# trungnt13/odin-ai

Hardware: AMD Instinct MI355X
Metric: VAE train images/sec (higher is better)
Workload: dtype f32; 1 GPU; dsprites_betavae_b256; global_batch=256, per_gpu_batch=256, parallelism=dp1, graph=True

## Files before the change

include/odin_hip.h:

```cpp
#ifndef ODIN_HIP_H
#define ODIN_HIP_H

#include <stddef.h>
#include <stdint.h>

#ifdef __cplusplus
extern "C" {
#endif

enum { ODIN_LINEAR = 0, ODIN_ELU = 1, ODIN_RELU = 2 };

typedef struct odin_conv_desc {
  int B, H, W, Cin;
  int OH, OW, Cout;
  int KH, KW, stride;
  int pad_t, pad_l;
  int act;
  int center;
  uint32_t* dy_amax;
  uint32_t* dx_amax;
  const uint32_t* x_amax;
  uint32_t* y_amax;
} odin_conv_desc;

// ... 36 lines not shown
                      const odin_conv_desc* d, void* stream);
int odin_conv2d_dgrad_first(const float* dy, const float* w, const float* aux, int aux_act, float* dx,
                            float* colsum_slab, int* colsum_rows_out, const odin_conv_desc* d, const float* x0,
                            float* wslab0, int* wslab0_rows_out, const odin_conv_desc* d0, void* stream);
int odin_dense_bwd(const float* x, const float* dy, const float* w, const float* aux, int aux_act, float* dx,
                   float* colsum_slab, int* colsum_rows_out, float* wslab, int* wslab_rows_out, int B, int K,
                   int N, int want_wgrad, int want_dgrad, const uint32_t* dy_amax, uint32_t* dx_amax, void* stream);
int odin_conv2d_reads_x_range(const odin_conv_desc* d);
int odin_deconv2d_reads_x_range(const odin_conv_desc* d);
int odin_dense_reads_x_range(int B, int K, int N);
int odin_dense_fwd_ranged(const float* x, const float* w, const float* bias, float* y, int B, int K, int N, int act,
                          const uint32_t* x_amax, uint32_t* y_amax, void* stream);
int odin_dense_bwd_ranged(const float* x, const float* dy, const float* w, const float* aux, int aux_act, float* dx,
                          float* colsum_slab, int* colsum_rows_out, float* wslab, int* wslab_rows_out, int B, int K,
                          int N, int want_wgrad, int want_dgrad, const uint32_t* dy_amax, uint32_t* dx_amax,
                          const uint32_t* x_amax, void* stream);
int odin_dense_dgrad_keeps_range(int B, int K, int N);

int odin_bernoulli_tail_fwd_bwd(int is_deconv, const float* x, const float* w, const float* bias,
                                const float* w1, const float* b1, const float* target,
                                float* logits, float* g_out, float* llk_part, int* n_part_out,
                                float* tail_slab, int* slab_rows_out, const float* scale,
                                const odin_conv_desc* d, int C1, void* stream);

int odin_dense_fwd(const float* x, const float* w, const float* bias, float* y, int B, int K,
                   int N, int act, void* stream);
int odin_dense_dgrad(const float* dy, const float* w, const float* aux, int aux_act, float* dx,
                     float* colsum_slab, int* slab_rows_out, int B, int K, int N, void* stream);
int odin_dense_wgrad(const float* x, const float* dy, float* slab, int* slab_rows_out, int B,
                     int K, int N, void* stream);

typedef struct odin_reduce_job {
  const float* src;
  float* dst;
  int n;
  int rows;
  int stride;
  int pad_;
} odin_reduce_job;
int odin_slab_reduce(const odin_reduce_job* jobs, int n_jobs, void* stream);

int odin_latent_fwd(const float* p, const float* eps, float* z, float* kl, float* fbmask, int B,
                    int D, int analytic, float free_bits, const float* capacity, void* stream);
int odin_latent_bwd(const float* p, const float* eps, const float* z, const float* dz,
                    const float* dz_extra, const float* fbmask, const float* klw,
                    const float* dloc_x, const float* dscale_x, float* dp, int B, int D,
// ... 232 lines not shown
```

odin_ai_amd/_lib.py:

```python
from __future__ import annotations

import ctypes as C
import os
from typing import Optional

_HERE = os.path.dirname(os.path.abspath(__file__))
DEFAULT_LIB = os.path.join(_HERE, 'libodin_hip.so')

ACT = {'linear': 0, 'elu': 1, 'relu': 2, None: 0}


class ConvDesc(C.Structure):
  _fields_ = [(n, C.c_int) for n in ('B', 'H', 'W', 'Cin', 'OH', 'OW', 'Cout', 'KH', 'KW',
                                     'stride', 'pad_t', 'pad_l', 'act', 'center')] + \
             [('dy_amax', C.c_void_p), ('dx_amax', C.c_void_p),
              ('x_amax', C.c_void_p), ('y_amax', C.c_void_p)]


class ReduceJob(C.Structure):
  _fields_ = [('src', C.c_void_p), ('dst', C.c_void_p), ('n', C.c_int), ('rows', C.c_int),
              ('stride', C.c_int), ('pad_', C.c_int)]


class AdamFold(C.Structure):
# ... 33 lines not shown
    'odin_dense_bwd': [P, P, P, P, I, P, P, IP, P, IP, I, I, I, I, I, P, P, P],
    'odin_dense_bwd_ranged': [P, P, P, P, I, P, P, IP, P, IP, I, I, I, I, I, P, P, P, P],
    'odin_dense_dgrad_keeps_range': [I, I, I],
    'odin_conv2d_reads_x_range': [DP],
    'odin_deconv2d_reads_x_range': [DP],
    'odin_dense_reads_x_range': [I, I, I],
    'odin_absmax': [P, C.c_size_t, P, P],
    'odin_debug_absmax_fallbacks': [],
    'odin_debug_stream_probe': [P, P, P, C.c_size_t, I, I, P],
    'odin_comm_unique_id': [P],
    'odin_comm_init': [C.POINTER(C.c_void_p), P, I, I],
    'odin_comm_destroy': [P],
    'odin_comm_library': [],
    'odin_allreduce_flat': [P, P, C.c_size_t, P],
    'odin_allgather_flat': [P, P, P, C.c_size_t, P],
    'odin_reduce_scatter_flat': [P, P, P, C.c_size_t, P],
    'odin_conv2d_fwd': [P, P, P, P, DP, P],
    'odin_conv2d_dgrad': [P, P, P, I, P, P, IP, DP, P],
    'odin_conv2d_wgrad': [P, P, P, IP, DP, P],
    'odin_deconv2d_fwd': [P, P, P, P, DP, P],
    'odin_deconv2d_dgrad': [P, P, P, I, P, P, IP, DP, P],
    'odin_deconv2d_wgrad': [P, P, P, IP, DP, P],
    'odin_bernoulli_tail_fwd_bwd': [I, P, P, P, P, P, P, P, P, P, IP, P, IP, P, DP, I, P],
    'odin_dense_fwd': [P, P, P, P, I, I, I, I, P],
    'odin_dense_fwd_ranged': [P, P, P, P, I, I, I, I, P, P, P],
    'odin_dense_dgrad': [P, P, P, I, P, P, IP, I, I, I, P],
    'odin_dense_wgrad': [P, P, P, IP, I, I, I, P],
    'odin_slab_reduce': [C.POINTER(ReduceJob), I, P],
    'odin_latent_fwd': [P, P, P, P, P, I, I, I, F, P, P],
    'odin_latent_bwd': [P, P, P, P, P, P, P, P, P, P, I, I, I, P],
    'odin_latent_tril_fwd': [P, P, P, P, P, I, I, I, F, P, P],
    'odin_latent_tril_bwd': [P, P, P, P, P, P, P, P, P, I, I, I, P],
    'odin_latent_tril_sample_logprob': [P, P, P, P, P, I, I, I, P],
    'odin_latent_block_rows': [I, I, I, I],
    'odin_latent_block_fwd': [P, P, P, P, P, C.c_uint64, P, P, P, P, P, P, P, P, I, I, I, I, I, I, F, P, P],
    'odin_latent_block_bwd': [P, P, P, P, P, P, P, P, P, P, P, P, I, P, P, P, P, P, I, I, I, I, I, P, P],
    'odin_wgrad_pair_begin': [],
    'odin_wgrad_pair_end': [],
    'odin_neck_rows': [I, I, I, I],
    'odin_neck_fwd': [C.POINTER(NeckArgs), P],
    'odin_neck_bwd': [C.POINTER(NeckArgs), P],
    'odin_elbo_bernoulli_fwd_bwd': [P, P, P, P, P, I, I, IP, P],
    'odin_elbo_bernoulli_fwd_bwd_ranged': [P, P, P, P, P, I, I, IP, P, P],
    'odin_elbo_gaussian_fwd_bwd': [P, P, P, P, P, I, I, I, I, IP, P],
    'odin_gaussian_tail_applicable': [DP, I],
    'odin_gaussian_tail_fwd_bwd': [P, P, P, P, P, P, P, P, P, IP, P, IP, P, DP, I, I, P],
# ... 155 lines not shown
```

odin_ai_amd/csrc/dispatch.hip:

```cpp
#include "odin_device.h"
#include "odin_internal.h"

namespace {

enum Family {
  GENERIC,
  SMALLC, PW1X1, SMALLDECONV, SMALLDECONV_GEN,
  FCONV_PLANES, FCONV_RING, FCONV_BLK, CONV5_BLK, TCONV_PLANES, TCONV_RING, TCONV_BLK, IGEMM_H, IGEMM,
  WGRAD_PLANES, WGRAD5_BLK, WGRAD_BLK, IGEMM_H_WGRAD, IGEMM_WGRAD,
  BWD_PLANES, BWD_BLK,
  TCONV_PLANES_FIRST,
  NOT_SERVED,
  BWD_PAIR,
  TINY_DENSE, THIN_DENSE, DENSE_H, DENSE_GEMM
};

enum { FOLDS_Y = 1, FOLDS_DX = 2, READS_X = 4 };
int traits(Family f) {
  switch (f) {
    case SMALLC: case SMALLDECONV_GEN: return FOLDS_Y;
    case SMALLDECONV: case IGEMM: case THIN_DENSE: return FOLDS_Y | FOLDS_DX;
    case FCONV_PLANES: case FCONV_BLK: case CONV5_BLK: case TCONV_PLANES: case TCONV_BLK: case IGEMM_H: case DENSE_H:
      return FOLDS_Y | FOLDS_DX | READS_X;
    case WGRAD_PLANES: case WGRAD5_BLK: case WGRAD_BLK: case IGEMM_H_WGRAD: return READS_X;
// ... 373 lines not shown
             ? 1 : 0;
}

extern "C" int odin_bernoulli_tail_fwd_bwd(int is_deconv, const float* x, const float* w, const float* bias, const float* w1,
                                           const float* b1, const float* target, float* logits, float* g_out,
                                           float* llk_part, int* n_part_out, float* tail_slab, int* slab_rows_out,
                                           const float* scale, const odin_conv_desc* d, int C1, void* stream) {
  const odin_geom g = odin_geom_fwd(d);
  const Family f = select_bernoulli_tail(is_deconv, g, d->act, C1);
  const odin_tail_args tail = {w1, b1, target, scale, logits, llk_part, tail_slab, C1};
  int rc;
  if (f == TCONV_PLANES)
    rc = odin_tconv_planes_launch(x, w, bias, nullptr, g_out, nullptr, slab_rows_out, w1, b1, target, logits, llk_part,
                                  n_part_out, tail_slab, scale, C1, d->B, d->H, d->W, d->Cin, d->Cout, 3, d->x_amax,
                                  d->dy_amax, stream);
  else if (f == TCONV_RING)
    rc = odin_tconv_ring_launch(x, w, bias, nullptr, g_out, nullptr, slab_rows_out, w1, b1, target, logits, llk_part,
                                n_part_out, tail_slab, scale, C1, d->B, d->H, d->W, d->Cout, 3, stream);
  else
    rc = odin_gather_generic(is_deconv, is_deconv ? 1 : 0, g, x, w, bias, d->act, nullptr, 0, g_out, nullptr,
                             -ODIN_MAX_COLSUM_BLOCKS, slab_rows_out, &tail, n_part_out, stream);
  return keep_range(rc, f, FOLDS_Y, g_out, (size_t)d->B * d->OH * d->OW * d->Cout, d->dy_amax, stream);
}
extern "C" int odin_bernoulli_tail_keeps_range(int is_deconv, const odin_conv_desc* d, int C1) {
  return (traits(select_bernoulli_tail(is_deconv, odin_geom_fwd(d), d->act, C1)) & FOLDS_Y) ? 1 : 0;
}

extern "C" int odin_dense_fwd(const float* x, const float* w, const float* bias, float* y, int B, int K, int N, int act,
                              void* stream) {
  return odin_dense_fwd_ranged(x, w, bias, y, B, K, N, act, nullptr, nullptr, stream);
}

extern "C" int odin_dense_fwd_ranged(const float* x, const float* w, const float* bias, float* y, int B, int K, int N,
                                     int act, const uint32_t* x_amax, uint32_t* y_amax, void* stream) {
  const Family f = select_dense_fwd(B, K, N, aligned16(x, w, y, bias));
  int rc;
  switch (f) {
    case TINY_DENSE: rc = odin_tiny_dense_fwd(x, w, bias, y, B, K, N, act, stream); break;
    case THIN_DENSE: rc = odin_thin_dense_fwd(x, w, bias, y, B, K, N, act, y_amax, stream); break;
    case DENSE_H: rc = odin_dense_h_fwd(x, w, bias, y, B, K, N, act, x_amax, y_amax, stream); break;
    case DENSE_GEMM: rc = odin_dense_gemm_fwd(x, w, bias, y, B, K, N, act, stream); break;
    default:
      rc = launch_gather(f, 0, 0, odin_geom_dense(B, K, N), x, w, bias, nullptr, 0, y, nullptr, nullptr, 1, act, nullptr,
                         y_amax, stream);
  }
  return keep_range(rc, f, FOLDS_Y, y, (size_t)B * N, y_amax, stream);
// ... 90 lines not shown
```

odin_ai_amd/csrc/odin_internal.h:

```cpp
#pragma once
#include <cstdio>
#include <cstring>
#include "../../include/odin_hip.h"

#define ODIN_MAX_SLAB_BLOCKS 256
#define ODIN_MAX_COLSUM_BLOCKS 512

#include <cstdlib>
#ifdef ODIN_DIAG
#define ODIN_DIAG_ENV(name) getenv(name)
#else
#define ODIN_DIAG_ENV(name) ((const char*)nullptr)
#endif
static inline bool odin_exact_fp32() { return getenv("ODIN_EXACT_FP32") != nullptr; }

struct odin_geom {
  int B, H, W, CI, OH, OW, CO, KH, KW, S, pt, pl, center;
};
static inline odin_geom odin_geom_fwd(const odin_conv_desc* d) {
  return {d->B, d->H, d->W, d->Cin, d->OH, d->OW, d->Cout, d->KH, d->KW, d->stride, d->pad_t, d->pad_l, d->center};
}
static inline odin_geom odin_geom_dgrad(const odin_conv_desc* d) {
  return {d->B, d->OH, d->OW, d->Cout, d->H, d->W, d->Cin, d->KH, d->KW, d->stride, d->pad_t, d->pad_l, 0};
}
// ... 95 lines not shown
                          int CO, int want_bias, int grad_u, const uint32_t* g_amax, const uint32_t* a_amax,
                          void* stream);
bool odin_conv5_blk_applicable(const odin_geom& g);
int odin_conv5_blk_launch(const float* in, const float* w, const float* bias, const float* aux, float* out,
                          float* colsum, int* rows_out, int B, int H, int W, int CI, int CO, int K, int epi, int act,
                          const uint32_t* in_amax, uint32_t* out_amax, void* stream);
bool odin_wgrad5_blk_applicable(const odin_geom& g);
int odin_wgrad5_blk_launch(const float* x, const float* dy, float* slab, int* rows_out, int B, int H, int W, int CI,
                           int CO, int K, int want_bias, const uint32_t* g_amax, const uint32_t* a_amax, void* stream);
bool odin_blk_enabled(double flop);
bool odin_blk_first();
bool odin_bwd_blk_applicable(const odin_geom& g);
int odin_bwd_blk_rows(const odin_geom& g);
int odin_bwd_blk_launch(const float* x, const float* dy, const float* w, const float* aux, int aux_act, float* dx,
                        float* colsum, float* wslab, int B, int H, int W, int Cin, int Cout, const uint32_t* dy_amax,
                        const uint32_t* x_amax, uint32_t* dx_amax, void* stream);
void odin_tconv_planes_set_stamps(void* buf);
bool odin_tconv_planes_applicable(const odin_geom& g, int epi, int C1);
int odin_tconv_planes_launch(const float* in, const float* w, const float* bias, const float* aux,
                             float* out, float* colsum, int* rows_out, const float* w1, const float* b1,
                             const float* target, float* logits, float* llk_part, int* n_part_out,
                             float* slab, const float* scale, int C1, int B, int H, int W, int CI,
                             int CO, int epi, const uint32_t* in_amax, uint32_t* out_amax, void* stream);
bool odin_tconv_planes_first_applicable(const odin_geom& g, const odin_geom& l0);
int odin_tconv_planes_first_launch(const float* in, const float* w, const float* aux, float* out, float* colsum, const float* img,
                                   int center0, float* wslab0, int* rows_out, int B, const uint32_t* in_amax,
                                   uint32_t* out_amax, void* stream);

bool odin_wgrad_planes_applicable(const odin_geom& g);
int odin_wgrad_planes_launch(const float* U, const float* V, float* slab, int* rows_out, int B, int OH,
                             int OW, int CI, int CO, int want_bias, int grad_u, const uint32_t* g_amax,
                             const uint32_t* a_amax, void* stream);

bool odin_fconv_planes_applicable(const odin_geom& g);
void odin_fconv_planes_set_stamps(void* buf);
int odin_fconv_planes_launch(const float* in, const float* w, const float* bias, const float* aux,
                             float* out, float* colsum, int* rows_out, int B, int OH, int OW, int CI, int CO,
                             int epi, const uint32_t* in_amax, uint32_t* out_amax, void* stream);

bool odin_igemm_applicable(int tmode, const odin_geom& g);
void odin_igemm_set_stamps(void* buf);
int odin_igemm_tiles(int tmode, const odin_geom& g);
int odin_igemm_launch(int tmode, const float* in, const float* w, const float* bias, const float* aux,
                      int aux_act, float* out, float* colsum, int B, int H, int W, int CI, int OH, int OW,
                      int CO, int KH, int KW, int S, int pt, int pl, int act, uint32_t* out_amax, void* stream);
void odin_igemm_pair_begin();
// ... 29 lines not shown
```

odin_ai_amd/csrc/tconv_planes.hip:

```cpp
#include "odin_device.h"
#include "odin_internal.h"
#include <cstdlib>
#include <utility>

namespace {

struct TPParams {
  const float* in;
  const float* w;
  const float* bias;
  const float* aux;
  float* out;
  float* colsum;
  const float* w1;
  const float* b1;
  const float* target;
  float* logits;
  float* llk_part;
  float* slab;
  const float* scale;
  int B, H, CO;
  int CS, ci_off;
  int tiles_per_img, n_tiles, tiles_per_wg;
  const unsigned* in_amax;
// ... 42 lines not shown

__device__ __forceinline__ float tp_pairsum32(float x) {
#ifdef ODIN_SIM
  return x + __shfl_xor(x, 32);
#else
  const unsigned u = __float_as_uint(x);
  const auto r = __builtin_amdgcn_permlane32_swap(u, u, false, false);
  return __uint_as_float(r[0]) + __uint_as_float(r[1]);
#endif
}

struct alignas(8) TpEnt {
  int x, y;
};

__host__ __device__ constexpr int tp_fw_addr(int lp, int n) {
  return (lp >> 1) * 256 + (((((lp & 1) << 3) + (n >> 2)) ^ ((lp >> 1) & 7)) << 4) + (n & 3) * 4;
}
constexpr int TP_FW_IMG_STRIDE = 72;
constexpr int TP_FW_IMG_FLOATS = 18 * TP_FW_IMG_STRIDE;
constexpr int TP_FW_BYTES = 8 * 4096 + TP_FW_IMG_FLOATS * 4;
static_assert(16 * 17 * 32 * 4 <= TP_FW_BYTES, "the partials of the 16 chains overlay the stage and the patch");

struct TpItem {
  float4 v;
  int dst;
  int ok;
};

template <int EPI, int C1, int W, int DBG = 0, bool ACC = false, int SCM = 0, bool PL = false, bool FW = false>
__device__ __forceinline__ void tp_body(const TPParams& p) {
  static_assert(!FW || (EPI == 2 && W == 16 && C1 == 1 && !ACC && !PL), "FW: the 32-channel data gradient, 16-pixel rows");
  constexpr int NPL = TP_NPL;
  constexpr int RP = 64 / W;
  constexpr int NSLOT = 2 * RP + 3;
  constexpr int PB = (W + 2) * 64;
  constexpr int RB = NPL * PB;
  constexpr int CPR = W / 8;
  constexpr int CSHIFT = (W == 32) ? 2 : (W == 16) ? 1 : 0;
  ODIN_DYN_SMEM(char, smem);
  char* wl = smem;
  char* ring = smem + TP_WBYTES;
  constexpr int NRED = 32 * (1 + (EPI == 3 ? C1 : 0)) + 4;
  __shared__ float cred[8 * NRED];
  __shared__ float llk_red[2][8];
  const int tid = threadIdx.x, lane = tid & 63;
#ifdef ODIN_SIM
  const int wave = tid >> 6;
#else
  const int wave = __builtin_amdgcn_readfirstlane(tid >> 6);
#endif
  const int l31 = lane & 31, half = lane >> 5;
  int stamp_i = 0;
  (void)stamp_i;
  TP_STAMP(1);
#if defined(ODIN_DIAG) && !defined(ODIN_SIM)
  if (p.stamps != nullptr && blockIdx.x == 0 && blockIdx.y == 0 && tid == 0) {
    p.stamps[64] = clock64();
    p.stamps[65] = wall_clock64();
  }
#endif
  const int n0 = blockIdx.y * 32;
  const int HP = p.H + 1;
  const int OH = 2 * p.H, OW = 2 * W;
  const int T0 = blockIdx.x * p.tiles_per_wg;
  int T1 = T0 + p.tiles_per_wg;
  if (T1 > p.n_tiles) T1 = p.n_tiles;
  if (T0 >= T1) return;

  const OdinRangeReq in_rq = odin_range_issue(SCM != 0 ? p.in_amax : nullptr, lane);
  float4 wv[8];
#pragma unroll
  for (int j = 0; j < 8; ++j) {
    const int e = tid + 512 * j;
    const int ci4 = e & 7, co = (e >> 3) & 31, tap = e >> 8;
    wv[j] = *reinterpret_cast<const float4*>(p.w + ((size_t)(tap * p.CO + n0 + co) * p.CS + p.ci_off + 4 * ci4));
  }
  const OdinRun IN = odin_run(p.in, (unsigned)((size_t)p.B * p.H * W * p.CS * 4));
  float amx = 0.f;
  const int f_c = wave & (CPR - 1), f_r0 = wave >> CSHIFT;
  constexpr int F_RJ = 8 >> CSHIFT;
  const int f_px = 8 * f_c + (lane >> 3), f_ch4 = lane & 7, f_pc = f_px + 1;
  const int f_lds_lane = f_pc * 64 + ((((f_ch4 >> 1) ^ ((f_pc >> 2) & 3))) << 4) + (f_ch4 & 1) * 8;
  const unsigned f_g_lane = (unsigned)((f_px * p.CS + p.ci_off + 4 * f_ch4) * 4);
  const unsigned f_rowbytes = (unsigned)(W * p.CS * 4);
  TpItem itA[2], itB[2];
  {
    const int tpi = p.tiles_per_img;
    const int b0 = odin_div_small(T0, tpi), t0 = T0 - b0 * tpi;
    const int start = HP * b0 + RP * t0;
#pragma unroll
    for (int j = 0; j < 2; ++j) {
      const int r = f_r0 + F_RJ * j, G = start + r;
// ... 116 lines not shown
#pragma unroll
    for (int r = 0; r < 16; ++r)
#pragma unroll
      for (int oc = 0; oc < C1; ++oc) {
        if (!CL) w1r[r][oc] = p.w1[(n0 + ch_of(r)) * C1 + oc];
        dw1[r][oc] = 0.f;
      }
#pragma unroll
    for (int oc = 0; oc < C1; ++oc) { b1r[oc] = p.b1[oc]; db1[oc] = 0.f; }
  }
  float csum[(EPI >= 2) ? 16 : 1];
#pragma unroll
  for (int r = 0; r < ((EPI >= 2) ? 16 : 1); ++r) csum[r] = 0.f;
  const float sc = (EPI == 3) ? p.scale[0] : 0.f;
  float llk_lane = 0.f;
  const unsigned out_bytes = (unsigned)((size_t)p.B * OH * OW * p.CO * 4);
  const OdinRun OUT = odin_run(p.out, out_bytes);
  const OdinRun AUX = odin_run(EPI == 2 ? p.aux : nullptr, EPI == 2 ? out_bytes : 0u);
  const unsigned tgt_bytes = (EPI == 3) ? (unsigned)((size_t)p.B * OH * OW * C1 * 4) : 0u;
  const OdinRun TG = odin_run(EPI == 3 ? p.target : nullptr, tgt_bytes);
  const OdinRun LG = odin_run(EPI == 3 ? p.logits : nullptr, (EPI == 3 && p.logits != nullptr) ? tgt_bytes : 0u);

  if (SCM != 0) {
    const unsigned in_mb = odin_range_finish(in_rq);
    scl = SCM == 1 || odin_act_needs_scale(in_mb);
    const int gk = scl ? odin_range_shift(in_mb) : 0;
    in_s = odin_pow2(gk); in_s2k = odin_pow2(gk + 11);
    out_s = odin_pow2(-gk); out_sx = odin_pow2(-gk - 11);
  }
  f32x16 biasv = f32x16_zero();
  if ((EPI == 1 || EPI == 3) && !CL) {
#pragma unroll
    for (int r = 0; r < 16; ++r) biasv[r] = bias_r[r] * in_s;
  }
  {
#pragma unroll
    for (int j = 0; j < 8; ++j) {
      const int e = tid + 512 * j;
      const int ci4 = e & 7, co = (e >> 3) & 31, tap = e >> 8;
      u32x2 h, l;
      odin_split_h4<false>(wv[j], 1.f, ODIN_LO_SCALE, h, l);
      char* d = wl + tap * TP_TAPB + (ci4 >> 1) * 512 + co * 16 + (ci4 & 1) * 8;
      *reinterpret_cast<u32x2*>(d) = h;
      *reinterpret_cast<u32x2*>(d + 2048) = l;
    }
  }
  store_fill(itA);
// ... 389 lines not shown
#pragma unroll
    for (int k = 0; k < N_EPI_OPS; ++k) epi_op(k);
  }
  flush_llk(T1 - 1);
  if (FW) {
    __syncthreads();
    fw_phase(t_cur);
    __syncthreads();
    float* part = reinterpret_cast<float*>(smem + p.fw_off);
#pragma unroll
    for (int r = 0; r < 16; ++r) {
      const int row = (r & 3) + 8 * (r >> 2) + 4 * fw_k;
      if (row <= 16) {
        part[(wave * 17 + row) * 32 + fw_j] = faccA[r];
        part[((wave + 8) * 17 + row) * 32 + fw_j] = faccB[r];
      }
    }
    __syncthreads();
    for (int e = tid; e < 17 * 32; e += 512) {
      float tt = 0.f;
#pragma unroll
      for (int c = 0; c < 16; c += 4)
        tt += (part[c * 544 + e] + part[(c + 1) * 544 + e]) + (part[(c + 2) * 544 + e] + part[(c + 3) * 544 + e]);
      p.wslab0[(size_t)blockIdx.x * (17 * 32) + e] = tt;
    }
  }

#if defined(ODIN_DIAG) && !defined(ODIN_SIM)
  if (p.stamps != nullptr && blockIdx.x == 0 && blockIdx.y == 0 && tid == 0) {
    p.stamps[66] = clock64();
    p.stamps[67] = wall_clock64();
  }
#endif
  if (EPI >= 1) {
    __syncthreads();
    odin_amax_commit_wg(p.out_amax, amx, tid, 512, cred, blockIdx.x + gridDim.x * blockIdx.y);
    __syncthreads();
  }
  if (EPI >= 2) {
#pragma unroll
    for (int r = 0; r < 16; ++r) {
      const int ch = (r & 3) + 8 * (r >> 2) + 4 * half;
      float vv = csum[r];
#pragma unroll
      for (int m = 16; m >= 1; m >>= 1) vv += __shfl_xor(vv, m);
      if (l31 == 0) cred[wave * NRED + ch] = vv;
      if (EPI == 3) {
#pragma unroll
        for (int oc = 0; oc < C1; ++oc) {
          float ww = dw1[r][oc];
#pragma unroll
          for (int m = 16; m >= 1; m >>= 1) ww += __shfl_xor(ww, m);
          if (l31 == 0) cred[wave * NRED + 32 + ch * C1 + oc] = ww;
        }
      }
    }
  }
  if (EPI == 3) {
#pragma unroll
    for (int oc = 0; oc < C1; ++oc) {
      float vv = db1[oc];
#pragma unroll
      for (int m = 16; m >= 1; m >>= 1) vv += __shfl_xor(vv, m);
      if (lane == 0) cred[wave * NRED + 32 + 32 * C1 + oc] = vv;
    }
  }
  if (EPI == 2 && p.colsum != nullptr) {
    __syncthreads();
    if (tid < 32) {
      float tt = 0.f;
      for (int wv = 0; wv < 8; ++wv) tt += cred[wv * NRED + tid];
      p.colsum[(size_t)blockIdx.x * p.CO + n0 + tid] = tt;
    }
  }
  if (EPI == 3) {
    __syncthreads();
    if (tid == 0) {
      const float* q = llk_red[(T1 - 1) & 1];
      p.llk_part[T1 - 1] = ((q[0] + q[1]) + (q[2] + q[3])) + ((q[4] + q[5]) + (q[6] + q[7]));
    }
    float* row = p.slab + (size_t)blockIdx.x * (p.CO * C1 + C1 + p.CO);
    for (int e = tid; e < 32 + 32 * C1 + C1; e += 512) {
      float tt = 0.f;
      for (int wv = 0; wv < 8; ++wv) tt += cred[wv * NRED + e];
      if (e < 32) {
        row[p.CO * C1 + C1 + e] = tt;
      } else if (e < 32 + 32 * C1) {
        const int ch = (e - 32) / C1, oc = (e - 32) - ch * C1;
        row[ch * C1 + oc] = tt;
      } else {
        row[p.CO * C1 + (e - 32 - 32 * C1)] = tt;
      }
    }
  }
}

template <int EPI, int C1, int W, int DBG = 0, bool ACC = false, int SCM = 0, bool FW = false>
__global__ __launch_bounds__(512) void tconv_planes_kernel(TPParams p) {
  tp_body<EPI, C1, W, DBG, ACC, SCM, false, FW>(p);
}

template <int EPI, int W, int SCM, bool PL>
__global__ __launch_bounds__(512) void tconv_planes2_kernel(TPParams p) {
  {
    TPParams q = p;
    q.colsum = nullptr;
    q.out_amax = nullptr;
    q.ci_off = 0;
    tp_body<0, 1, W, 0, false, SCM, PL>(q);
  }
  odin_wait_vmem();
#ifndef ODIN_SIM
  __builtin_amdgcn_fence(__ATOMIC_SEQ_CST, "workgroup");
#endif
  __syncthreads();
  p.ci_off = 32;
  tp_body<EPI, 1, W, 0, true, SCM, PL>(p);
}

constexpr int TP_LDS_MAX = 152 * 1024;
int tp_ring_bytes(int W) { return TP_WBYTES + (2 * (64 / W) + 3) * TP_NPL * (W + 2) * 64; }
int tp_fill_bytes(int W) { return 8 * 2 * (W == 32 ? 2 : W == 16 ? 4 : 8); }
int tp_tiles_per_wg(int W, int n_tiles, int gy, int extra_lds = 0) {
  int cap = odin_num_cus() / gy;
  if (cap < 1) cap = 1;
  if (cap > ODIN_MAX_COLSUM_BLOCKS) cap = ODIN_MAX_COLSUM_BLOCKS;
  int tpw = (n_tiles + cap - 1) / cap;
  const int limit = (TP_LDS_MAX - extra_lds - tp_ring_bytes(W)) / tp_fill_bytes(W) - 3;
  if (tpw > limit) tpw = limit;
  if ((n_tiles + tpw - 1) / tpw > ODIN_MAX_COLSUM_BLOCKS) return -1;
  return tpw;
}

template <int EPI, int C1, bool ACC, int SC>
int tp_launch_w(const TPParams& p, int W, dim3 grid, void* stream) {
  const size_t lds = (size_t)tp_ring_bytes(W) + (size_t)(p.tiles_per_wg + 3) * tp_fill_bytes(W);
  constexpr int W3 = (EPI == 3 ? 16 : 8);
#ifndef ODIN_SIM
  static bool attr_done = false;
  if (!attr_done) {
// ... 65 lines not shown
  if (PL) {
    lds = (lds + 15) & ~(size_t)15;
    p.part_off = (int)lds;
    lds += (size_t)p.tiles_per_wg * 32768;
  }
#ifndef ODIN_SIM
  static bool attr_done = false;
  if (!attr_done) {
    const void* fns[3] = {reinterpret_cast<const void*>(&tconv_planes2_kernel<EPI, 32, SC, PL>),
                          reinterpret_cast<const void*>(&tconv_planes2_kernel<EPI, 16, SC, PL>),
                          reinterpret_cast<const void*>(&tconv_planes2_kernel<EPI, 8, SC, PL>)};
    for (int i = 0; i < 3; ++i)
      if (hipFuncSetAttribute(fns[i], hipFuncAttributeMaxDynamicSharedMemorySize, TP2_LDS_MAX) != hipSuccess)
        (void)hipGetLastError();
    attr_done = true;
  }
#endif
  if (W == 32) ODIN_LAUNCH((tconv_planes2_kernel<EPI, 32, SC, PL>), grid, dim3(512), lds, stream, p);
  else if (W == 16) ODIN_LAUNCH((tconv_planes2_kernel<EPI, 16, SC, PL>), grid, dim3(512), lds, stream, p);
  else ODIN_LAUNCH((tconv_planes2_kernel<EPI, 8, SC, PL>), grid, dim3(512), lds, stream, p);
  return odin_check_launch("tconv_planes(f16x2)");
}

}

static long long* g_tp_stamps = nullptr;
void odin_tconv_planes_set_stamps(void* buf) { g_tp_stamps = (long long*)buf; }

bool odin_tconv_planes_applicable(const odin_geom& g, int epi, int C1) {
  const int B = g.B, H = g.H, W = g.W, CI = g.CI, CO = g.CO, KH = g.KH, KW = g.KW, S = g.S, pt = g.pt, pl = g.pl;
  if (odin_blk_first()) return false;
  if (odin_exact_fp32() || ODIN_DIAG_ENV("ODIN_NOPLANES") || ODIN_DIAG_ENV("ODIN_SPLIT")) return false;
  if (epi == 3 && (CO != 32 || (C1 != 1 && C1 != 3) || CI != 32 || W == 8)) return false;
  return KH == 4 && KW == 4 && S == 2 && pt == 1 && pl == 1 && (CI == 32 || CI == 64) && (CO % 32) == 0 &&
         !g.center && (W == 8 || W == 16 || W == 32) && (H % (64 / W)) == 0 && (size_t)B * H * W * CI * 4 < (1ull << 31) &&
         (size_t)B * H * W * 4 * C1 * 4 < (1ull << 31) && tp_tiles_per_wg(W, B * (H / (64 / W)), CO / 32) > 0;
}

int odin_tconv_planes_launch(const float* in, const float* w, const float* bias, const float* aux,
                             float* out, float* colsum, int* rows_out, const float* w1, const float* b1,
                             const float* target, float* logits, float* llk_part, int* n_part_out,
                             float* slab, const float* scale, int C1, int B, int H, int W, int CI,
                             int CO, int epi, const uint32_t* in_amax, uint32_t* out_amax, void* stream) {
  TPParams p;
  memset(&p, 0, sizeof(p));
  p.in = in; p.w = w; p.bias = bias; p.aux = aux; p.out = out; p.colsum = colsum;
// ... 87 lines not shown
```

odin_ai_amd/engine.py:

```python
from __future__ import annotations

import ctypes as C
import math
from typing import Callable, Dict, List, NamedTuple, Optional, Sequence, Tuple

import numpy as np
import torch

from . import _lib
from ._lib import ACT, ConvDesc, ReduceJob


def same_pads(n: int, k: int, s: int) -> Tuple[int, int, int]:
  out = -(-n // s)
  total = max((out - 1) * s + k - n, 0)
  return out, total // 2, total - total // 2


class ParamLayout:

  def __init__(self):
    self.entries: List[Tuple[tuple, Tuple[int, ...], int]] = []
    self.size = 0

# ... 381 lines not shown

  def ptr(self) -> Optional[int]:
    return None if self.value is None else self.value.data_ptr()


class VAEEngine:

  def __init__(self, enc_layers, dec_layers, in_shape, zdim, batch_size, device,
               observation='bernoulli', analytic=False, free_bits=None, tc=None, lib=None,
               params: Optional[torch.Tensor] = None, world_size: int = 1, seed: int = 1,
               optim_state: Optional[Tuple[torch.Tensor, torch.Tensor]] = None,
               force_dp: bool = False, reverse: bool = True, capacity: bool = False,
               range_words: Optional[torch.Tensor] = None, *,
               act_words: bool = True, hyper_ring: bool = True, hyper_ring_rows: int = 128, fuse_norm: bool = True,
               overlap_wgrad: Optional[str] = None, early_reduce: bool = False, defer_wgrad: bool = False,
               fuse_first_wgrad: bool = True, side_streams: int = 2, small_wgrad_gf: float = 0.8, dp_buckets: Optional[int] = None,
               neck: bool = True, neck_bwd: Optional[bool] = None, static_top_word: bool = True,
               latent_reg: Optional[str] = None, reg_coef: float = 1.0, mmd_kernel: str = 'gaussian',
               mmd_prior_samples: int = 100, dip_lambda: Tuple[float, float] = (1.0, 2.0), prior_seed: int = 0,
               vamprior_components: Optional[int] = None, pseudoinputs_mean: float = -0.05,
               pseudoinputs_std: float = 0.01, pseudoinputs=None,
               vq_codes: Optional[int] = None, vq_code_size: Optional[int] = None, vq_commitment: float = 0.25,
               vq_ema: bool = False, vq_ema_decay: float = 0.99, vq_epsilon: float = 1e-5, vq_state=None,
               latent_cov: str = 'diag'):
    self.lib = lib if lib is not None else _lib.load()
    self.device = torch.device(device)
    self.B, self.D = int(batch_size), int(zdim)
    self.capacity_on = bool(capacity)
    self.in_shape = tuple(in_shape)
    self.observation = observation
    if latent_cov not in ('diag', 'tril'):
      raise ValueError(f"latent_cov={latent_cov!r}: expected 'diag' or 'tril'")
    self.latent_cov = latent_cov
    self.set_kl_form(analytic, reverse)
    self.free_bits = -1.0 if free_bits is None else float(free_bits)
    self.tc_mode, self.world_size, self.seed = tc, int(world_size), int(seed)
    self.is_dp = self.world_size > 1 or bool(force_dp)
    self.tc_sharded = tc == 'betatc' and self.is_dp
    if latent_reg not in (None, 'mmd', 'dip_i', 'dip_ii'):
      raise ValueError(f"latent_reg={latent_reg!r}: expected None, 'mmd', 'dip_i' or 'dip_ii'")
    if latent_reg is not None and tc is not None:
      raise ValueError(f'latent_reg={latent_reg!r} cannot be combined with tc={tc!r}')
    if latent_reg == 'mmd' and mmd_kernel not in MMD_KERNELS:
      raise NotImplementedError(f'mmd_kernel={mmd_kernel!r}: the HIP path offers {sorted(MMD_KERNELS)}')
    self.reg_mode, self.reg_coef = latent_reg, float(reg_coef)
    self.reg_sharded = latent_reg is not None and self.is_dp
    self.vamp_K = None if vamprior_components is None else int(vamprior_components)
# ... 83 lines not shown
    self.n_part = 0
    if self.vq_K is None:
      rows = C.c_int(0)
      self.lib.odin_dense_wgrad(None, None, None, C.byref(rows), B, self.hdim, self.pw, None)
      self.lat_slab = torch.empty(rows.value, self.hdim * self.pw + self.pw, **f32)
      self.lat_rows = rows.value
    if tc == 'betatc':
      self.tc_ws = torch.zeros(self.lib.odin_total_correlation_workspace(
          B, B * self.world_size if self.tc_sharded else B, D), **f32)
      self.tc_dz = torch.empty(B, D, **f32)
      self.tc_dloc = torch.empty(B, D, **f32)
      self.tc_dscale = torch.empty(B, D, **f32)
      if self.tc_sharded:
        Bg = B * self.world_size
        self.tc_pz_local = torch.empty(B, 3 * D, **f32)
        self.tc_pz_all = torch.empty(Bg, 3 * D, **f32)
        self.tc_p_all = torch.empty(Bg, 2 * D, **f32)
        self.tc_part_all = torch.empty(2, Bg, D, **f32)
    if latent_reg is not None:
      self._plan_latent_reg(f32, mmd_kernel, mmd_prior_samples, dip_lambda, prior_seed)
    if self.vq_K is None:
      self._plan_fused_tail(f32)
      self._plan_gauss_head(f32)
      if latent_cov == 'tril':
        self._plan_tril(bool(act_words))
      else:
        self._plan_latent_block(f32)
        self._neck_bwd_opt = neck_bwd
        self._plan_neck(f32, bool(neck))
    else:
      self._plan_vq(f32, own_params, vq_state)
    if self.vamp_K is not None:
      self._plan_vamprior(f32, mr, act_words, small_wgrad_gf)
    self._term = self._plan_term()
    self.ws = torch.empty(4096, **f32)
    self.gnorm2 = torch.zeros(1, **f32)
    self.flag = torch.zeros(1, dtype=torch.int32, device=self.device)
    self.skip_hit = torch.zeros(1, dtype=torch.int32, device=self.device)
    self.skipped_update = torch.zeros(1, dtype=torch.int32, device=self.device)
    offs = [o for _, _, o in self.layout.entries] + [self.n_params_end()]
    self.seg_offsets = torch.tensor(offs, dtype=torch.int64, device=self.device)
    self._ring = [torch.zeros(N_HYPER + 4, dtype=torch.float32) for _ in range(8)]
    self._ring_ev = [None] * 8
    if self.device.type == 'cuda':
      self._ring = [t.pin_memory() for t in self._ring]
    self._ring_i = 0
# ... 283 lines not shown
    ne, nl = len(self.enc_recs), len(self.enc_recs) + len(self.dec_recs)
    self._tril_dp_word = self.range_words.data_ptr() + 4 * RANGE_WORDS * 2 * nl
    self._tril_x_word = None
    if act_words and self.lib.odin_dense_reads_x_range(self.B, self.hdim, self.pw):
      self._tril_x_word = self.enc.y_word[ne - 1] = self.enc.aword(ne - 1)
      if self.enc.descs[ne - 1] is not None:
        self.enc.descs[ne - 1].y_amax = self._tril_x_word

  def _resolve_vq_code_size(self, code_size):
    H, K = self.hdim, self.vq_K
    Cs = H if code_size is None else int(code_size)
    if Cs < 1 or H % Cs != 0:
      raise ValueError(f'vq_code_size={code_size}: must divide the encoder output width {H}')
    if Cs > 256 or K * Cs * 4 > 64 * 1024 or self.B * (H // Cs) > 65536:
      raise ValueError(f'vq_codes={K}, vq_code_size={Cs}, batch_size={self.B}: outside the quantiser kernel '
                       f'(Cs <= 256, K * Cs * 4 B <= 64 KB, B * L <= 65536)')
    if self.enc_recs[-1].kind == 'deconv':
      raise NotImplementedError('vq_codes: an encoder that ends in a Conv2DTranspose is not offered')
    self.vq_Cs, self.vq_L = Cs, H // Cs

  def _plan_vq(self, f32, own_params, vq_state):
    K, Cs, L, B = self.vq_K, self.vq_Cs, self.vq_L, self.B
    self.fused_tail, self.tail_mode = False, None
    self.gauss_head = self._used_head = False
    self.lat_block = self._used_block = False
    self.neck = self._used_neck = False
    self._neck_bwd_opt = None
    self.vq_N = B * L
    i32 = dict(dtype=torch.int32, device=self.device)
    self.vq_idx = torch.zeros(self.vq_N, **i32)
    self.vq_cnt = torch.zeros(K, **i32)
    self.vq_ws = torch.zeros(self.lib.odin_vq_workspace(self.vq_N), **f32)
    assert self.vq_ws.data_ptr() % 8 == 0
    if self.vq_ema:
      if vq_state is not None:
        self.vq_codebook, self.vq_ema_counts, self.vq_ema_means = vq_state
        assert tuple(self.vq_codebook.shape) == (K, Cs) and tuple(self.vq_ema_means.shape) == (K, Cs)
      else:
        self.vq_codebook = torch.empty(K, Cs, **f32)
        self.vq_ema_means = torch.empty(K, Cs, **f32)
        self.vq_ema_counts = torch.empty(K, **f32)
        self.init_codebook()
      self.vq_dcb = None
    else:
      assert vq_state is None, 'vq_state belongs to vq_ema=True: the codebook is a parameter otherwise'
      self.vq_codebook = self.params[self.vq_cb_off:self.vq_cb_off + K * Cs].view(K, Cs)
# ... 69 lines not shown
    if self.observation != 'bernoulli' or len(recs) < 2:
      return
    a, b = recs[-2], recs[-1]
    if not (b.kind == 'conv' and b.desc['K'] == 1 and b.desc['stride'] == 1 and b.act == 'linear'
            and b.desc['Cout'] <= 4 and a.kind in ('conv', 'deconv') and a.desc['Cout'] <= 32):
      return
    rows, npart = C.c_int(0), C.c_int(0)
    try:
      self.lib.odin_bernoulli_tail_fwd_bwd(int(a.kind == 'deconv'), None, None, None, None, None,
                                           None, None, None, None, C.byref(npart), None,
                                           C.byref(rows), None, C.byref(self.dec.descs[-2]),
                                           b.desc['Cout'], None)
    except _lib.OdinError:
      return
    if a.desc['OH'] * a.desc['OW'] <= 128:
      return
    self.fused_tail = True
    self.tail_keeps_range = bool(self.lib.odin_bernoulli_tail_keeps_range(
        int(a.kind == 'deconv'), C.byref(self.dec.descs[-2]), b.desc['Cout']))
    self.tail_rows, self.tail_npart = rows.value, npart.value
    co, c1 = a.desc['Cout'], b.desc['Cout']
    self.tail_slab = torch.empty(rows.value, co * c1 + c1 + co, **f32)
    self.tail_llk_part = torch.empty(self.B * npart.value, **f32)

  def _plan_gauss_tail(self, f32):
    a, b = self.dec_recs[-2], self.dec_recs[-1]
    Cc = self.in_shape[-1]
    if not (b.kind == 'conv' and b.desc['K'] == 1 and b.desc['stride'] == 1 and b.act == 'linear'
            and b.desc['Cout'] == 2 * Cc and a.kind == 'deconv'):
      return
    d = self.dec.descs[-2]
    if not self.lib.odin_gaussian_tail_applicable(C.byref(d), Cc):
      return
    rows, npart = C.c_int(0), C.c_int(0)
    self.lib.odin_gaussian_tail_fwd_bwd(None, None, None, None, None, None, None, None, None, C.byref(npart), None,
                                        C.byref(rows), None, C.byref(d), Cc, OBS_MODE[self.observation], None)
    self.fused_tail = True
    self.tail_mode = OBS_MODE[self.observation]
    self.tail_keeps_range = True
    self.tail_rows, self.tail_npart = rows.value, npart.value
    co, c1 = a.desc['Cout'], b.desc['Cout']
    self.tail_slab = torch.empty(rows.value, co * c1 + c1 + co, **f32)
    self.tail_llk_part = torch.empty(self.B * npart.value, **f32)

  def _plan_gauss_head(self, f32):
    self.gauss_head = self._used_head = False
# ... 370 lines not shown
      self.dec.descs[nd2].dy_amax = self.dec.word(nd2)
    self._used_head = False
    if self.gauss_head:
      nd2 = len(self.dec_recs) - 2
      self.dec.set_top_word(True, nd2)
    if self.gauss_head and fused:
      nd = len(self.dec_recs)
      hm = self.dec.forward(dec_in, st, upto=nd - 1, start=dec_start)
      a, b = self.dec_recs[-2], self.dec_recs[-1]
      Cc = self.in_shape[-1]
      rows = C.c_int(0)
      lib.odin_gaussian_head_fwd_bwd(
          hm.data_ptr(), self.dec.w(nd - 1).data_ptr(), self.dec.b(nd - 1).data_ptr(), x.data_ptr(),
          self.dec.outs[-1].data_ptr(), None, self.dec.gouts[-2].data_ptr(), self.head_llk_part.data_ptr(),
          C.byref(npart), self.head_slab.data_ptr(), C.byref(rows),
          self.head_colsum.data_ptr() if self.head_colsum is not None else None, self.hp(H_INVB), B,
          self.n_per // Cc, b.desc['Cin'], Cc, self.head_mode, ACT[a.act], self.dec.word(nd - 2), st)
      assert rows.value == self.head_rows and npart.value == self.head_npart
      self._used_fused, self._used_head = False, True
      llk_part = self.head_llk_part
      h_d = self.dec.outs[-1]
    elif self.fused_tail and fused:
      nd = len(self.dec_recs)
      h = self.dec.forward(dec_in, st, upto=nd - 2, start=dec_start)
      a, b = self.dec_recs[-2], self.dec_recs[-1]
      rows = C.c_int(0)
      if self.tail_mode is not None:
        lib.odin_gaussian_tail_fwd_bwd(
            h.data_ptr(), self.dec.w(nd - 2).data_ptr(), self.dec.b(nd - 2).data_ptr(),
            self.dec.w(nd - 1).data_ptr(), self.dec.b(nd - 1).data_ptr(), x.data_ptr(),
            self.dec.outs[-1].data_ptr(), self.dec.gouts[-2].data_ptr(), self.tail_llk_part.data_ptr(),
            C.byref(npart), self.tail_slab.data_ptr(), C.byref(rows), self.hp(H_INVB),
            C.byref(self.dec.descs[-2]), self.in_shape[-1], self.tail_mode, st)
        assert rows.value == self.tail_rows and npart.value == self.tail_npart
      else:
        lib.odin_bernoulli_tail_fwd_bwd(
            int(a.kind == 'deconv'), h.data_ptr(), self.dec.w(nd - 2).data_ptr(),
            self.dec.b(nd - 2).data_ptr(), self.dec.w(nd - 1).data_ptr(),
            self.dec.b(nd - 1).data_ptr(), x.data_ptr(), self.dec.outs[-1].data_ptr(),
            self.dec.gouts[-2].data_ptr(), self.tail_llk_part.data_ptr(), C.byref(npart),
            self.tail_slab.data_ptr(), C.byref(rows), self.hp(H_INVB), C.byref(self.dec.descs[-2]),
            b.desc['Cout'], st)
      self._used_fused = True
      llk_part = self.tail_llk_part
      h_d = self.dec.outs[-1]
    else:
      self._used_fused = False
      llk_part = self.llk_part
      h_d = self.dec.forward(dec_in, st, start=dec_start)
    if not (self._used_fused or self._used_head):
# ... 482 lines not shown
```

Baseline: 567,300 images/sec.

## Chain the last decoder deconv into the fused Bernoulli tail kernel

Adds a single kernel that runs the 16x16→32x32 deconv (both 32-channel halves) and then the fused Bernoulli tail deconv+1x1+loss in the same workgroups. Each workgroup handles whole images, so the intermediate activation's range is kept in shared memory and there is no separate launch or global amax round-trip between the two layers. The engine uses the chain by default when the shapes match and the row and partition layout equals the existing tail's. The cost is a coarser grid, one workgroup per group of images capped at the CU count, which may lower occupancy and parallelism for the first stage.

```diff
diff --git a/include/odin_hip.h b/include/odin_hip.h
--- a/include/odin_hip.h
+++ b/include/odin_hip.h
@@ -82,6 +82,12 @@
                                 float* logits, float* g_out, float* llk_part, int* n_part_out,
                                 float* tail_slab, int* slab_rows_out, const float* scale,
                                 const odin_conv_desc* d, int C1, void* stream);
+
+int odin_decoder_tail_chain(const float* x, const float* w3, const float* b3, float* y3, const odin_conv_desc* d3,
+                            const float* w4, const float* b4, const float* w1, const float* b1, const float* target,
+                            float* logits, float* g_out, float* llk_part, int* n_part_out, float* tail_slab,
+                            int* slab_rows_out, int* same_partition_out, const float* scale, const odin_conv_desc* d4,
+                            int C1, void* stream);
 
 int odin_dense_fwd(const float* x, const float* w, const float* bias, float* y, int B, int K,
                    int N, int act, void* stream);
diff --git a/odin_ai_amd/_lib.py b/odin_ai_amd/_lib.py
--- a/odin_ai_amd/_lib.py
+++ b/odin_ai_amd/_lib.py
@@ -79,6 +79,7 @@
     'odin_deconv2d_dgrad': [P, P, P, I, P, P, IP, DP, P],
     'odin_deconv2d_wgrad': [P, P, P, IP, DP, P],
     'odin_bernoulli_tail_fwd_bwd': [I, P, P, P, P, P, P, P, P, P, IP, P, IP, P, DP, I, P],
+    'odin_decoder_tail_chain': [P, P, P, P, DP, P, P, P, P, P, P, P, P, IP, P, IP, IP, P, DP, I, P],
     'odin_dense_fwd': [P, P, P, P, I, I, I, I, P],
     'odin_dense_fwd_ranged': [P, P, P, P, I, I, I, I, P, P, P],
     'odin_dense_dgrad': [P, P, P, I, P, P, IP, I, I, I, P],
diff --git a/odin_ai_amd/csrc/dispatch.hip b/odin_ai_amd/csrc/dispatch.hip
--- a/odin_ai_amd/csrc/dispatch.hip
+++ b/odin_ai_amd/csrc/dispatch.hip
@@ -419,6 +419,19 @@
                              -ODIN_MAX_COLSUM_BLOCKS, slab_rows_out, &tail, n_part_out, stream);
   return keep_range(rc, f, FOLDS_Y, g_out, (size_t)d->B * d->OH * d->OW * d->Cout, d->dy_amax, stream);
 }
+extern "C" int odin_decoder_tail_chain(const float* x, const float* w3, const float* b3, float* y3, const odin_conv_desc* d3,
+                                       const float* w4, const float* b4, const float* w1, const float* b1,
+                                       const float* target, float* logits, float* g_out, float* llk_part, int* n_part_out,
+                                       float* tail_slab, int* slab_rows_out, int* same_partition_out, const float* scale,
+                                       const odin_conv_desc* d4, int C1, void* stream) {
+  const odin_geom g3 = odin_geom_fwd(d3), g4 = odin_geom_fwd(d4);
+  if (select_deconv2d_fwd(g3, true, d3->act) != TCONV_PLANES || select_bernoulli_tail(1, g4, d4->act, C1) != TCONV_PLANES ||
+      !odin_tconv_chain2_applicable(g3, g4, C1))
+    return odin_fail(-2, "decoder_tail_chain: shapes outside the chain");
+  return odin_tconv_chain2_launch(x, w3, b3, y3, w4, b4, w1, b1, target, logits, g_out, llk_part, n_part_out, tail_slab,
+                                  slab_rows_out, same_partition_out, scale, C1, d3->B, d3->x_amax, d3->y_amax, d4->dy_amax,
+                                  stream);
+}
 extern "C" int odin_bernoulli_tail_keeps_range(int is_deconv, const odin_conv_desc* d, int C1) {
   return (traits(select_bernoulli_tail(is_deconv, odin_geom_fwd(d), d->act, C1)) & FOLDS_Y) ? 1 : 0;
 }
diff --git a/odin_ai_amd/csrc/odin_internal.h b/odin_ai_amd/csrc/odin_internal.h
--- a/odin_ai_amd/csrc/odin_internal.h
+++ b/odin_ai_amd/csrc/odin_internal.h
@@ -141,6 +141,12 @@
                              const float* target, float* logits, float* llk_part, int* n_part_out,
                              float* slab, const float* scale, int C1, int B, int H, int W, int CI,
                              int CO, int epi, const uint32_t* in_amax, uint32_t* out_amax, void* stream);
+bool odin_tconv_chain2_applicable(const odin_geom& g3, const odin_geom& g4, int C1);
+int odin_tconv_chain2_launch(const float* x, const float* w3, const float* b3, float* y3, const float* w4, const float* b4,
+                             const float* w1, const float* b1, const float* target, float* logits, float* g_out,
+                             float* llk_part, int* n_part_out, float* slab, int* rows_out, int* same_partition_out,
+                             const float* scale, int C1, int B, const uint32_t* x_amax, uint32_t* y3_amax,
+                             uint32_t* dy_amax, void* stream);
 bool odin_tconv_planes_first_applicable(const odin_geom& g, const odin_geom& l0);
 int odin_tconv_planes_first_launch(const float* in, const float* w, const float* aux, float* out, float* colsum, const float* img,
                                    int center0, float* wslab0, int* rows_out, int B, const uint32_t* in_amax,
diff --git a/odin_ai_amd/csrc/tconv_planes.hip b/odin_ai_amd/csrc/tconv_planes.hip
--- a/odin_ai_amd/csrc/tconv_planes.hip
+++ b/odin_ai_amd/csrc/tconv_planes.hip
@@ -88,6 +88,39 @@
 constexpr int TP_FW_BYTES = 8 * 4096 + TP_FW_IMG_FLOATS * 4;
 static_assert(16 * 17 * 32 * 4 <= TP_FW_BYTES, "the partials of the 16 chains overlay the stage and the patch");
 
+struct TpAt {
+  int n0;
+  int T0;
+  int row;
+  int slot;
+  const unsigned* in_local;
+  unsigned* out_local;
+};
+
+__device__ __forceinline__ unsigned tp_uniform(unsigned v) {
+#ifdef ODIN_SIM
+  return v;
+#else
+  return __builtin_amdgcn_readfirstlane(v);
+#endif
+}
+__device__ __forceinline__ TpAt tp_here(const TPParams& p) {
+  return TpAt{(int)blockIdx.y * 32, (int)blockIdx.x * p.tiles_per_wg, -1, -1, nullptr, nullptr};
+}
+__device__ __forceinline__ void tp_amax_commit_local(unsigned* block, unsigned* local, float amx, int tid, float* red,
+                                                     unsigned wg) {
+  const float m = odin_wave_max64(amx);
+  if ((tid & 63) == 0) red[tid >> 6] = m;
+  __syncthreads();
+  if (tid == 0) {
+    float t = red[0];
+    for (int w = 1; w < 8; ++w) t = fmaxf(t, red[w]);
+    const unsigned b = odin_fbits(t);
+    if (block != nullptr) atomicMax(block + (wg & (ODIN_RANGE_SLOTS - 1)) * ODIN_RANGE_STRIDE, b);
+    if (b > *local) *local = b;
+  }
+}
+
 struct TpItem {
   float4 v;
   int dst;
@@ -95,7 +128,7 @@
 };
 
 template <int EPI, int C1, int W, int DBG = 0, bool ACC = false, int SCM = 0, bool PL = false, bool FW = false>
-__device__ __forceinline__ void tp_body(const TPParams& p) {
+__device__ __forceinline__ void tp_body(const TPParams& p, const TpAt at) {
   static_assert(!FW || (EPI == 2 && W == 16 && C1 == 1 && !ACC && !PL), "FW: the 32-channel data gradient, 16-pixel rows");
   constexpr int NPL = TP_NPL;
   constexpr int RP = 64 / W;
@@ -126,15 +159,16 @@
     p.stamps[65] = wall_clock64();
   }
 #endif
-  const int n0 = blockIdx.y * 32;
+  const int n0 = at.n0;
+  auto wg_row = [&] { return at.row < 0 ? (size_t)blockIdx.x : (size_t)at.row; };
   const int HP = p.H + 1;
   const int OH = 2 * p.H, OW = 2 * W;
-  const int T0 = blockIdx.x * p.tiles_per_wg;
+  const int T0 = at.T0;
   int T1 = T0 + p.tiles_per_wg;
   if (T1 > p.n_tiles) T1 = p.n_tiles;
   if (T0 >= T1) return;
 
-  const OdinRangeReq in_rq = odin_range_issue(SCM != 0 ? p.in_amax : nullptr, lane);
+  const OdinRangeReq in_rq = odin_range_issue((SCM != 0 && at.in_local == nullptr) ? p.in_amax : nullptr, lane);
   float4 wv[8];
 #pragma unroll
   for (int j = 0; j < 8; ++j) {
@@ -297,7 +331,7 @@
   const OdinRun LG = odin_run(EPI == 3 ? p.logits : nullptr, (EPI == 3 && p.logits != nullptr) ? tgt_bytes : 0u);
 
   if (SCM != 0) {
-    const unsigned in_mb = odin_range_finish(in_rq);
+    const unsigned in_mb = at.in_local != nullptr ? tp_uniform(*at.in_local) : odin_range_finish(in_rq);
     scl = SCM == 1 || odin_act_needs_scale(in_mb);
     const int gk = scl ? odin_range_shift(in_mb) : 0;
     in_s = odin_pow2(gk); in_s2k = odin_pow2(gk + 11);
@@ -733,7 +767,7 @@
 #pragma unroll
       for (int c = 0; c < 16; c += 4)
         tt += (part[c * 544 + e] + part[(c + 1) * 544 + e]) + (part[(c + 2) * 544 + e] + part[(c + 3) * 544 + e]);
-      p.wslab0[(size_t)blockIdx.x * (17 * 32) + e] = tt;
+      p.wslab0[wg_row() * (17 * 32) + e] = tt;
     }
   }
 
@@ -745,7 +779,9 @@
 #endif
   if (EPI >= 1) {
     __syncthreads();
-    odin_amax_commit_wg(p.out_amax, amx, tid, 512, cred, blockIdx.x + gridDim.x * blockIdx.y);
+    const unsigned slot = at.slot < 0 ? blockIdx.x + gridDim.x * blockIdx.y : (unsigned)at.slot;
+    if (at.out_local != nullptr) tp_amax_commit_local(p.out_amax, at.out_local, amx, tid, cred, slot);
+    else odin_amax_commit_wg(p.out_amax, amx, tid, 512, cred, slot);
     __syncthreads();
   }
   if (EPI >= 2) {
@@ -781,7 +817,7 @@
     if (tid < 32) {
       float tt = 0.f;
       for (int wv = 0; wv < 8; ++wv) tt += cred[wv * NRED + tid];
-      p.colsum[(size_t)blockIdx.x * p.CO + n0 + tid] = tt;
+      p.colsum[wg_row() * p.CO + n0 + tid] = tt;
     }
   }
   if (EPI == 3) {
@@ -790,7 +826,7 @@
       const float* q = llk_red[(T1 - 1) & 1];
       p.llk_part[T1 - 1] = ((q[0] + q[1]) + (q[2] + q[3])) + ((q[4] + q[5]) + (q[6] + q[7]));
     }
-    float* row = p.slab + (size_t)blockIdx.x * (p.CO * C1 + C1 + p.CO);
+    float* row = p.slab + wg_row() * (p.CO * C1 + C1 + p.CO);
     for (int e = tid; e < 32 + 32 * C1 + C1; e += 512) {
       float tt = 0.f;
       for (int wv = 0; wv < 8; ++wv) tt += cred[wv * NRED + e];
@@ -808,7 +844,7 @@
 
 template <int EPI, int C1, int W, int DBG = 0, bool ACC = false, int SCM = 0, bool FW = false>
 __global__ __launch_bounds__(512) void tconv_planes_kernel(TPParams p) {
-  tp_body<EPI, C1, W, DBG, ACC, SCM, false, FW>(p);
+  tp_body<EPI, C1, W, DBG, ACC, SCM, false, FW>(p, tp_here(p));
 }
 
 template <int EPI, int W, int SCM, bool PL>
@@ -818,7 +854,7 @@
     q.colsum = nullptr;
     q.out_amax = nullptr;
     q.ci_off = 0;
-    tp_body<0, 1, W, 0, false, SCM, PL>(q);
+    tp_body<0, 1, W, 0, false, SCM, PL>(q, tp_here(q));
   }
   odin_wait_vmem();
 #ifndef ODIN_SIM
@@ -826,7 +862,32 @@
 #endif
   __syncthreads();
   p.ci_off = 32;
-  tp_body<EPI, 1, W, 0, true, SCM, PL>(p);
+  tp_body<EPI, 1, W, 0, true, SCM, PL>(p, tp_here(p));
+}
+
+template <int C1>
+__global__ __launch_bounds__(512) void tconv_chain2_kernel(TPParams p3, TPParams pt) {
+  __shared__ unsigned y_local;
+  if (threadIdx.x == 0) y_local = 0u;
+  auto stage_sync = [] {
+    odin_wait_vmem();
+#ifndef ODIN_SIM
+    __builtin_amdgcn_fence(__ATOMIC_SEQ_CST, "workgroup");
+#endif
+    __syncthreads();
+  };
+  const int T3 = (int)blockIdx.x * p3.tiles_per_wg;
+  {
+    TPParams q = p3;
+    q.out_amax = nullptr;
+    q.ci_off = 0;
+    tp_body<0, 1, 16, 0, false, 2, false>(q, TpAt{0, T3, 0, 0, nullptr, nullptr});
+  }
+  stage_sync();
+  p3.ci_off = 32;
+  tp_body<1, 1, 16, 0, true, 2, false>(p3, TpAt{0, T3, 0, (int)blockIdx.x, nullptr, &y_local});
+  stage_sync();
+  tp_body<3, C1, 32, 0, false, 2>(pt, TpAt{0, (int)blockIdx.x * pt.tiles_per_wg, (int)blockIdx.x, (int)blockIdx.x, &y_local, nullptr});
 }
 
 constexpr int TP_LDS_MAX = 152 * 1024;
@@ -938,6 +999,70 @@
   return odin_check_launch("tconv_planes(f16x2)");
 }
 
+int tp_chain_ipw(int B) {
+  int cap = odin_num_cus();
+  if (cap > ODIN_MAX_COLSUM_BLOCKS) cap = ODIN_MAX_COLSUM_BLOCKS;
+  if (cap < 1) cap = 1;
+  return (B + cap - 1) / cap;
+}
+
+template <int C1>
+int tp_launch_chain2(const TPParams& p3, const TPParams& pt, int gx, size_t lds, void* stream) {
+#ifndef ODIN_SIM
+  static size_t attr_lds = 0;
+  if (lds > attr_lds) {
+    if (hipFuncSetAttribute(reinterpret_cast<const void*>(&tconv_chain2_kernel<C1>),
+                            hipFuncAttributeMaxDynamicSharedMemorySize, (int)lds) != hipSuccess)
+      (void)hipGetLastError();
+    attr_lds = lds;
+  }
+#endif
+  ODIN_LAUNCH((tconv_chain2_kernel<C1>), dim3(gx, 1, 1), dim3(512), lds, stream, p3, pt);
+  return odin_check_launch("tconv_chain2(f16x2)");
+}
+
+}
+
+bool odin_tconv_chain2_applicable(const odin_geom& g3, const odin_geom& g4, int C1) {
+  if (!odin_tconv_planes_applicable(g3, 1, 1) || !odin_tconv_planes_applicable(g4, 3, C1)) return false;
+  if (g3.B != g4.B || g3.H != 16 || g3.W != 16 || g3.CI != 64 || g3.CO != 32 || g4.H != 32 || g4.W != 32 || g4.CI != 32 ||
+      g4.CO != 32)
+    return false;
+  const int ipw = tp_chain_ipw(g3.B);
+  return (size_t)tp_ring_bytes(32) + (size_t)(16 * ipw + 3) * tp_fill_bytes(32) <= (size_t)TP_LDS_MAX &&
+         (size_t)tp_ring_bytes(16) + (size_t)(4 * ipw + 3) * tp_fill_bytes(16) <= (size_t)TP_LDS_MAX;
+}
+
+int odin_tconv_chain2_launch(const float* x, const float* w3, const float* b3, float* y3, const float* w4, const float* b4,
+                             const float* w1, const float* b1, const float* target, float* logits, float* g_out,
+                             float* llk_part, int* n_part_out, float* slab, int* rows_out, int* same_partition_out,
+                             const float* scale, int C1, int B, const uint32_t* x_amax, uint32_t* y3_amax,
+                             uint32_t* dy_amax, void* stream) {
+  const int ipw = tp_chain_ipw(B), gx = (B + ipw - 1) / ipw;
+  if (rows_out) *rows_out = gx;
+  if (n_part_out) *n_part_out = 16;
+  if (same_partition_out) *same_partition_out = tp_tiles_per_wg(32, B * 16, 1) == 16 * ipw ? 1 : 0;
+  if (y3 == nullptr) return 0;
+  TPParams p3, pt;
+  memset(&p3, 0, sizeof(p3));
+  memset(&pt, 0, sizeof(pt));
+  p3.in = x; p3.w = w3; p3.bias = b3; p3.out = y3;
+  p3.B = B; p3.H = 16; p3.CO = 32; p3.CS = 64;
+  p3.tiles_per_img = 4; p3.n_tiles = 4 * B;
+  p3.tiles_per_wg = 4 * ipw;
+  p3.in_amax = x_amax; p3.out_amax = y3_amax;
+  const size_t lds3 = (size_t)tp_ring_bytes(16) + (size_t)(p3.tiles_per_wg + 3) * tp_fill_bytes(16);
+  pt.in = y3; pt.w = w4; pt.bias = b4; pt.out = g_out;
+  pt.w1 = w1; pt.b1 = b1; pt.target = target; pt.logits = logits; pt.llk_part = llk_part; pt.slab = slab; pt.scale = scale;
+  pt.B = B; pt.H = 32; pt.CO = 32; pt.CS = 32;
+  pt.tiles_per_img = 16; pt.n_tiles = 16 * B; pt.tiles_per_wg = 16 * ipw;
+  pt.out_amax = dy_amax;
+  const size_t ldst = (size_t)tp_ring_bytes(32) + (size_t)(pt.tiles_per_wg + 3) * tp_fill_bytes(32);
+  const size_t lds = lds3 > ldst ? lds3 : ldst;
+  if (lds > (size_t)TP_LDS_MAX) return odin_fail(-2, "tconv_chain2: LDS");
+  if (C1 == 1) return tp_launch_chain2<1>(p3, pt, gx, lds, stream);
+  if (C1 == 3) return tp_launch_chain2<3>(p3, pt, gx, lds, stream);
+  return odin_fail(-2, "tconv_chain2: one or three logit maps only");
 }
 
 static long long* g_tp_stamps = nullptr;
diff --git a/odin_ai_amd/engine.py b/odin_ai_amd/engine.py
--- a/odin_ai_amd/engine.py
+++ b/odin_ai_amd/engine.py
@@ -427,7 +427,7 @@
                pseudoinputs_std: float = 0.01, pseudoinputs=None,
                vq_codes: Optional[int] = None, vq_code_size: Optional[int] = None, vq_commitment: float = 0.25,
                vq_ema: bool = False, vq_ema_decay: float = 0.99, vq_epsilon: float = 1e-5, vq_state=None,
-               latent_cov: str = 'diag'):
+               latent_cov: str = 'diag', chain_fwd: bool = True):
     self.lib = lib if lib is not None else _lib.load()
     self.device = torch.device(device)
     self.B, self.D = int(batch_size), int(zdim)
@@ -557,6 +557,7 @@
     if self.vq_K is None:
       self._plan_fused_tail(f32)
       self._plan_gauss_head(f32)
+      self._plan_chain_fwd(bool(chain_fwd))
       if latent_cov == 'tril':
         self._plan_tril(bool(act_words))
       else:
@@ -886,6 +887,7 @@
   def _plan_vq(self, f32, own_params, vq_state):
     K, Cs, L, B = self.vq_K, self.vq_Cs, self.vq_L, self.B
     self.fused_tail, self.tail_mode = False, None
+    self.chain_tail = False
     self.gauss_head = self._used_head = False
     self.lat_block = self._used_block = False
     self.neck = self._used_neck = False
@@ -1001,6 +1003,24 @@
     co, c1 = a.desc['Cout'], b.desc['Cout']
     self.tail_slab = torch.empty(rows.value, co * c1 + c1 + co, **f32)
     self.tail_llk_part = torch.empty(self.B * npart.value, **f32)
+
+  def _plan_chain_fwd(self, want: bool):
+    self.chain_tail = False
+    recs = self.dec_recs
+    if not (want and self.fused_tail and self.tail_mode is None and not self.is_dp and len(recs) >= 3 and
+            recs[-3].kind == 'deconv' and recs[-2].kind == 'deconv'):
+      return
+    d3 = recs[-3].desc
+    if (d3['H'], d3['W'], d3['Cin'], d3['Cout'], d3['K'], d3['stride']) != (16, 16, 64, 32, 4, 2):
+      return
+    rows, npart, same = C.c_int(0), C.c_int(0), C.c_int(0)
+    try:
+      self.lib.odin_decoder_tail_chain(None, None, None, None, C.byref(self.dec.descs[-3]), None, None, None, None, None,
+                                       None, None, None, C.byref(npart), None, C.byref(rows), C.byref(same), None,
+                                       C.byref(self.dec.descs[-2]), recs[-1].desc['Cout'], None)
+    except _lib.OdinError:
+      return
+    self.chain_tail = bool(same.value) and rows.value == self.tail_rows and npart.value == self.tail_npart
 
   def _plan_gauss_tail(self, f32):
     a, b = self.dec_recs[-2], self.dec_recs[-1]
@@ -1417,10 +1437,18 @@
       h_d = self.dec.outs[-1]
     elif self.fused_tail and fused:
       nd = len(self.dec_recs)
-      h = self.dec.forward(dec_in, st, upto=nd - 2, start=dec_start)
+      chain = self.chain_tail and dec_start <= nd - 3 and not self.debug_check_ranges
+      h = self.dec.forward(dec_in, st, upto=nd - 3 if chain else nd - 2, start=dec_start)
       a, b = self.dec_recs[-2], self.dec_recs[-1]
       rows = C.c_int(0)
-      if self.tail_mode is not None:
+      if chain:
+        lib.odin_decoder_tail_chain(
+            h.data_ptr(), self.dec.w(nd - 3).data_ptr(), self.dec.b(nd - 3).data_ptr(), self.dec.outs[nd - 3].data_ptr(),
+            C.byref(self.dec.descs[nd - 3]), self.dec.w(nd - 2).data_ptr(), self.dec.b(nd - 2).data_ptr(),
+            self.dec.w(nd - 1).data_ptr(), self.dec.b(nd - 1).data_ptr(), x.data_ptr(), self.dec.outs[-1].data_ptr(),
+            self.dec.gouts[-2].data_ptr(), self.tail_llk_part.data_ptr(), C.byref(npart), self.tail_slab.data_ptr(),
+            C.byref(rows), None, self.hp(H_INVB), C.byref(self.dec.descs[-2]), b.desc['Cout'], st)
+      elif self.tail_mode is not None:
         lib.odin_gaussian_tail_fwd_bwd(
             h.data_ptr(), self.dec.w(nd - 2).data_ptr(), self.dec.b(nd - 2).data_ptr(),
             self.dec.w(nd - 1).data_ptr(), self.dec.b(nd - 1).data_ptr(), x.data_ptr(),
```

After: 580,000 images/sec (median of 6 runs). +2.2%, better.
